# ruizhecao96/CMGAN

Measured on AMD Instinct MI355X. Metric: enhanced audio frames/sec (16 kHz, 2 s clips, batch 32 per GPU), higher is better.
Workload: dtype f32 storage/accumulate; products as 3 x f16 split MFMA (fp32-class accuracy); 1 GPU; configs[1]: batch=32 x 2 s synthetic 16 kHz noisy clips per GPU, n_fft=400 hop=100, TSCNet(64,201) random-init, full pipeline wav->wav; mfma_mode=f16x3, launch=hipGraph replay, batch_per_gpu=32, global_batch=32, frames_per_clip=321, parallelism=dp1

## Files before the change

cmgan_amd/csrc/api.hip:

```cpp
#include <math.h>
#include <stdarg.h>
#include <stdio.h>
#include <string.h>

#include <algorithm>
#include <map>
#include <string>
#include <vector>

#include "api_internal.h"
#include "weights.h"

extern "C" void cmgan_default_config(cmgan_config* c) {
    if (!c) return;
    c->n_fft = 400; c->hop = 100; c->num_features = 201; c->num_channel = 64; c->num_tscb = 4;
    c->heads = 4; c->dim_head = 16; c->conv_kernel = 31; c->max_pos_emb = 512;
    c->mfma_mode = CMGAN_MFMA_F16X3;
    c->single_mask = 0;
}

extern "C" int cmgan_abi_version(void) { return CMGAN_ABI_VERSION; }

extern "C" const char* cmgan_last_error(const cmgan_handle* h) {
    return h ? h->err.c_str() : g_create_error.c_str();
// ... 494 lines not shown
    w.qkv_w = W(h, WID(g, CF_QKV_W), ok);   w.qkv_b = W(h, WID(g, CF_QKV_B), ok);
    w.wo = W(h, WID(g, CF_WO), ok);         w.bo = W(h, WID(g, CF_BO), ok);
    w.rel = W(h, WID(g, CF_REL), ok);
    w.pw1_w = W(h, WID(g, CF_PW1_W), ok);   w.pw1_b = W(h, WID(g, CF_PW1_B), ok);
    w.dw_w = W(h, WID(g, CF_DW_W), ok);     w.dw_b = W(h, WID(g, CF_DW_B), ok);
    w.pw2_w = W(h, WID(g, CF_PW2_W), ok);   w.pw2_b = W(h, WID(g, CF_PW2_B), ok);
    w.ff2_w1 = W(h, WID(g, CF_FF2_W1), ok); w.ff2_b1 = W(h, WID(g, CF_FF2_B1), ok);
    w.ff2_w2 = W(h, WID(g, CF_FF2_W2), ok); w.ff2_b2 = W(h, WID(g, CF_FF2_B2), ok);
    w.post_gb = W(h, WID(g, CF_POST_GB), ok);
    w.max_pos = h->cfg.max_pos_emb;
    return ok;
}

#ifndef CX_IMG
#define CX_IMG 1
#endif
#ifndef CX_NIMG
#define CX_NIMG 1
#endif
struct WsPlan {
    size_t total = 0;
    size_t e[5];
    size_t img[3];
    size_t xa, xb, q, k, v, o, u, w;
    size_t dm, dc;
    size_t partials;
    size_t ns;
    size_t mstat;
    size_t scale;
    size_t spec;
    size_t est;
    size_t frames;
};

static size_t take(size_t& cur, size_t n) {
    const size_t o = cur;
    cur += (n + 63) & ~(size_t)63;
    return o;
}

static WsPlan plan_ws(const cmgan_config& c, int B, int T) {
    WsPlan p;
    const size_t F = c.num_features, F2 = (F + 1) / 2, W2 = 2 * F2;
    const size_t P = (size_t)T * F, P2 = (size_t)T * F2, M = (size_t)B * P2;
    size_t cur = 0;
    p.e[0] = take(cur, (size_t)B * T * std::max(F, W2) * 64);
    for (int i = 1; i < 5; ++i) p.e[i] = take(cur, (size_t)B * P * 64);
    for (int i = 0; i < 3; ++i)
        p.img[i] = (CX_IMG && c.mfma_mode != CMGAN_MFMA_F32 && i < CX_NIMG) ? take(cur, (size_t)B * P * 64) : 0;
    p.xa = take(cur, M * 64);
    p.xb = take(cur, M * 64);
    const size_t qf = std::max(conf_qkv_floats((int)(B * F2), T), conf_qkv_floats(B * T, (int)F2));
    p.q = take(cur, qf); p.k = take(cur, qf); p.v = take(cur, qf); p.o = take(cur, qf);
    p.u = take(cur, M * 128);
    p.w = take(cur, M * 128);
    p.dm = take(cur, (size_t)B * T * W2 * 4 + 64);
    p.dc = take(cur, (size_t)B * T * W2 * 4 + 64);
    const size_t nt = std::max({(size_t)conv3_ntiles(T, (int)F), (size_t)conv_in_ntiles((int)P),
                                (size_t)conv3x_ntiles(T, (int)F, 64), (size_t)conv3x_ntiles(T, (int)F, 128)});
    p.partials = take(cur, (size_t)B * nt * 128 * 2);
    p.ns = take(cur, (size_t)16 * 2 * B * 64);
    p.mstat = take(cur, (size_t)B * 2);
    p.scale = take(cur, (size_t)B);
    p.spec = take(cur, (size_t)B * 2 * P);
    p.est = take(cur, (size_t)B * 2 * P);
    p.frames = take(cur, (size_t)B * T * c.n_fft);
    p.total = cur;
    return p;
}

extern "C" size_t cmgan_workspace_bytes(const cmgan_handle* h, int B, int T) {
    if (!h || B <= 0 || T <= 0) return 0;
    return plan_ws(h->cfg, B, T).total * sizeof(float);
}

extern "C" int cmgan_num_frames(const cmgan_handle* h, int L) { return h ? L / h->cfg.hop + 1 : 0; }

static int check_wave_len(cmgan_handle* h, int L, bool whole_hops) {
// ... 24 lines not shown
    if (!h) return CMGAN_E_BADARG;
    if (!re || !im || !wav_out || B <= 0 || T < 2) return fail(h, CMGAN_E_BADARG, "cmgan_uncompress_istft: bad argument");
    const WsPlan p = plan_ws(h->cfg, B, T);
    if (int rc = check_ws(h, ws, ws_bytes, p.total * sizeof(float))) return rc;
    launch_uncompress_istft(begin(h, stream), h->st, re, im, scale, B, T, (float*)ws + p.frames, wav_out);
    return check_launch(h, "uncompress_istft");
}

extern "C" int cmgan_power_compress(cmgan_handle* h, const float* x, int B, int F, int T, float* y, void* stream) {
    if (!h) return CMGAN_E_BADARG;
    if (!x || !y || B <= 0 || F <= 0 || T <= 0) return fail(h, CMGAN_E_BADARG, "cmgan_power_compress: bad argument");
    launch_power_compress(begin(h, stream), x, B, F, T, y);
    return check_launch(h, "power_compress");
}

extern "C" int cmgan_power_uncompress(cmgan_handle* h, const float* re, const float* im, int B, int F, int T,
                                      float* y, void* stream) {
    if (!h) return CMGAN_E_BADARG;
    if (!re || !im || !y || B <= 0 || F <= 0 || T <= 0) return fail(h, CMGAN_E_BADARG, "cmgan_power_uncompress: bad argument");
    launch_power_uncompress(begin(h, stream), re, im, B, F, T, y);
    return check_launch(h, "power_uncompress");
}

struct ConfPlan { size_t total, xa, xb, q, k, v, o, u, w; };
static ConfPlan plan_conf(int N, int L) {
    ConfPlan p;
    size_t cur = 0;
    const size_t M = (size_t)N * L, qf = conf_qkv_floats(N, L);
    p.xa = take(cur, M * 64); p.xb = take(cur, M * 64);
    p.q = take(cur, qf); p.k = take(cur, qf); p.v = take(cur, qf); p.o = take(cur, qf);
    p.u = take(cur, M * 128); p.w = take(cur, M * 128);
    p.total = cur;
    return p;
}

extern "C" size_t cmgan_conformer_workspace_bytes(const cmgan_handle* h, int N, int L) {
    if (!h || N <= 0 || L <= 0) return 0;
    return plan_conf(N, L).total * sizeof(float);
}

static int conformer_forward_impl(cmgan_handle* h, int index, const float* x, int N, int L, const unsigned char* mask,
                                  float* y, float* taps, void* ws, size_t ws_bytes, void* stream);

static bool conformer_mix(cmgan_handle* h, LaunchCtx ctx, const ConfWeights& w, const ConfWeightsX3& w16, const ConfBuffers& b,
                          const TokMap& seq, long M, float* taps, bool outer_residual, const unsigned char* mask) {
    const int sm = h->cfg.single_mask;
    if (sm == 0) return conformer_forward_x3(ctx, w, w16, b, seq, M, taps, outer_residual, mask);
    if (sm == CMGAN_MIX_ALL || (sm | CMGAN_MIX_CONV) == CMGAN_MIX_ALL)
        return conformer_forward_x1(ctx, w, w16, b, seq, M, taps, outer_residual, mask);
    if (!conformer_x3_addressable(seq)) return false;
    const ConfStageTbl &t3 = conf_stages_x3(), &t1 = conf_stages_x1();
    auto pick = [&](int bit) -> const ConfStageTbl& { return (sm & bit) ? t1 : t3; };
    return conformer_forward_tbl(ctx, pick(CMGAN_MIX_FF1), pick(CMGAN_MIX_QKV), pick(CMGAN_MIX_ATTN), pick(CMGAN_MIX_PW1),
                                 pick(CMGAN_MIX_DWPW2), pick(CMGAN_MIX_FF2), w, w16, b, seq, M, taps, outer_residual, mask);
// ... 5 lines not shown
}

extern "C" int cmgan_conformer_forward_masked(cmgan_handle* h, int index, const float* x, int N, int L,
                                              const unsigned char* mask, float* y, float* taps, void* ws,
                                              size_t ws_bytes, void* stream) {
    if (h && !mask) return fail(h, CMGAN_E_BADARG, "cmgan_conformer_forward_masked: mask is null");
    return conformer_forward_impl(h, index, x, N, L, mask, y, taps, ws, ws_bytes, stream);
}

static int conformer_forward_impl(cmgan_handle* h, int index, const float* x, int N, int L, const unsigned char* mask,
                                  float* y, float* taps, void* ws, size_t ws_bytes, void* stream) {
    if (!h) return CMGAN_E_BADARG;
    if (!x || !y || N <= 0 || L <= 0 || index < 0 || index >= 8) return fail(h, CMGAN_E_BADARG, "cmgan_conformer_forward: bad argument");
    if ((long)N * L >= (1l << 31)) return fail(h, CMGAN_E_BADARG, "cmgan_conformer_forward: N x L too large");
    const TokMap seq = make_seq_map(N, L, 1, L, 0, 1);
    if (h->cfg.mfma_mode != CMGAN_MFMA_F32 && !conformer_x3_addressable(seq))
        return fail(h, CMGAN_E_BADARG, "cmgan_conformer_forward: N x L too large for the split-f16 kernels "
                                       "(L < 2^23, N * ceil(L / 32) < 2^31)");
    const ConfPlan p = plan_conf(N, L);
    if (int rc = check_ws(h, ws, ws_bytes, p.total * sizeof(float))) return rc;
    ConfWeights w;
    if (!conf_weights(h, index, w)) return CMGAN_E_WEIGHTS;
    float* f = (float*)ws;
    ConfBuffers b{f + p.xa, f + p.xb, f + p.q, f + p.k, f + p.v, f + p.o, f + p.u, f + p.w};
    hipStream_t s = (hipStream_t)stream;
    const size_t M = (size_t)N * L;
    HIPCHK(h, hipMemcpyAsync(b.xa, x, M * 64 * sizeof(float), hipMemcpyDeviceToDevice, s));
    if (h->cfg.mfma_mode != CMGAN_MFMA_F32) {
        ConfWeightsX3 w16;
        if (!conf_weights_x3(h, index, w16)) return CMGAN_E_WEIGHTS;
        if (!conformer_mix(h, begin(h, stream), w, w16, b, seq, (long)M, taps, false, mask))
            return fail(h, CMGAN_E_BADARG, "cmgan_conformer_forward: N x L too large for the split-f16 kernels");
    } else {
        conformer_forward(begin(h, stream), w, b, seq, (long)M, taps, false, mask);
    }
    HIPCHK(h, hipMemcpyAsync(y, b.xa, M * 64 * sizeof(float), hipMemcpyDeviceToDevice, s));
    return check_launch(h, "conformer_forward");
}

struct DenseW { const float *w[4], *bias[4], *gb[4], *prelu[4]; const _Float16* w16[4]; };
static bool dense_weights(cmgan_handle* h, int grp, DenseW& d) {
    bool ok = true;
    for (int i = 0; i < 4; ++i) {
        d.w[i] = W(h, WID(grp, DB_W(i)), ok); d.bias[i] = W(h, WID(grp, DB_BIAS(i)), ok);
        d.gb[i] = W(h, WID(grp, DB_GB(i)), ok); d.prelu[i] = W(h, WID(grp, DB_PRELU(i)), ok);
        d.w16[i] = W16(h, WID(grp, DB_W(i)), ok);
    }
// ... 137 lines not shown
    {
        float* slots[4] = {f + p.e[1], f + p.e[2], f + p.e[3], f + p.e[4]};
        float* sc[4] = {nsc(1), nsc(2), nsc(3), nsc(4)};
        float* sh[4] = {nsh(1), nsh(2), nsh(3), nsh(4)};
        float* imgs[3] = {f + p.img[0], f + p.img[1], f + p.img[2]};
        run_dense_block(ctx, x3, dbe, f + p.e[0], nsc(0), nsh(0), c1pr, slots, partials, sc, sh, B, T, F, x3 ? imgs : nullptr, conv3x, frozen,
                        run, 1);
    }
    {
        ConvArgs a{};
        a.in[0] = f + p.e[4]; a.nscale[0] = nsc(4); a.nshift[0] = nsh(4); a.nalpha[0] = dbe.prelu[3];
        a.nslots = 1; a.w = c2w; a.bias = c2b; a.out = f + p.xb; a.partials = partials;
        a.T = T; a.F = F; a.dil = 1; a.mode = 1; a.ntiles = x3 ? conv3x_ntiles(T, F, 64) : conv3_ntiles(T, F);
        if (x3) conv3x(ctx, a, c2w16, B, 1, 64);
        else launch_conv3(ctx, a, B, 1, 64);
        finalize(5, a.ntiles, 64, 0, (double)P2, c2gb, f + p.xb, F2);
        launch_in_apply(ctx, f + p.xb, nsc(5), nsh(5), c2pr, f + p.xa, B, P2);
    }
    if (taps && taps->encoder_dev) launch_cl_to_nchw(ctx, f + p.xa, taps->encoder_dev, B, P2);
    }
    const size_t x_bytes = (size_t)M * 64 * sizeof(float);
    if (opt.x_io && !ph_enc) HIPCHK(h, hipMemcpyAsync(f + p.xa, opt.x_io, x_bytes, hipMemcpyDeviceToDevice, hs));

    ConfBuffers cb{f + p.xa, f + p.xb, f + p.q, f + p.k, f + p.v, f + p.o, f + p.u, f + p.w};
    const TokMap tmap = make_seq_map(B * F2, T, F2, (long)T * F2, 1, F2);
    const TokMap fmap = make_seq_map(B * T, F2, 1, F2, 0, 1);
    for (int k = 0; ph_tscb && k < h->cfg.num_tscb; ++k) {
        if (x3) {
            if (!conformer_x(ctx, cw[2 * k], cw16[2 * k], cb, tmap, M, nullptr, true, nullptr) ||
                !conformer_x(ctx, cw[2 * k + 1], cw16[2 * k + 1], cb, fmap, M, nullptr, true, nullptr))
                return fail(h, CMGAN_E_BADARG, "tscnet_forward: B x T x F too large for the split-f16 conformer kernels "
                                               "(conformer_x3_addressable, conformer_x3.hip)");
        } else {
            conformer_forward(ctx, cw[2 * k], cb, tmap, M, nullptr, true);
            conformer_forward(ctx, cw[2 * k + 1], cb, fmap, M, nullptr, true);
        }
        if (taps && taps->tscb_dev[k]) launch_cl_to_nchw(ctx, f + p.xa, taps->tscb_dev[k], B, P2);
    }

    if (opt.x_io && !ph_dec) HIPCHK(h, hipMemcpyAsync(opt.x_io, f + p.xa, x_bytes, hipMemcpyDeviceToDevice, hs));
    const size_t enc_floats = (size_t)6 * 2 * B * 64;
    if (!ph_dec) {
        if (opt.stats_out && ph_enc)
            HIPCHK(h, hipMemcpyAsync(opt.stats_out, f + p.ns, enc_floats * sizeof(float), hipMemcpyDeviceToDevice, hs));
        return check_launch(h, "tscnet_forward");
    }

// ... 303 lines not shown
```

cmgan_amd/csrc/attn32_x3.hip:

```cpp
#if defined(X3_SINGLE) && defined(A32_STAMP)
#undef A32_STAMP
#endif
#include "kernels.h"
#include <string.h>
#include <stdlib.h>

namespace X3_NS {

typedef float f32x16 __attribute__((ext_vector_type(16)));

__device__ __forceinline__ f32x16 mfma3216(f16x8 a, f16x8 b, f32x16 c) {
    return __builtin_amdgcn_mfma_f32_32x32x16_f16(a, b, c, 0, 0, 0);
}
__device__ __forceinline__ f32x16 mfma3216l(f16x8 a, f16x8 b, f32x16 c) {
    return X3_TERMS == 3 ? __builtin_amdgcn_mfma_f32_32x32x16_f16(a, b, c, 0, 0, 0) : c;
}
__device__ __forceinline__ f32x16 zero16() {
    f32x16 z;
#pragma unroll
    for (int i = 0; i < 16; ++i) z[i] = 0.f;
    return z;
}
#ifdef A32_STAMP
#define A32_SLOTS 2048
// ... 32 lines not shown
    const float a = xchg32(v, b);
    return a + b;
}

#ifndef XCD_ORDER
#define XCD_ORDER 1
#endif
#define XNTB 2
#define XWAVES 8

__device__ __forceinline__ void ln_split32(const f32x4 (&x)[4], f16x8 (&bh)[2], f16x8 (&bl)[2]) {
    float mean, rstd;
    ln_stats(x, mean, rstd);
    f32x4 xh[4];
#pragma unroll
    for (int kb = 0; kb < 4; ++kb) xh[kb] = (x[kb] - splat4(mean)) * splat4(rstd);
    split8(xh[0], xh[1], bh[0], bl[0]);
    split8(xh[2], xh[3], bh[1], bl[1]);
}

__global__ __launch_bounds__(512) void qkv32_x3_kernel(const float* __restrict__ x, TokMap m, int Lt,
                                                       const _Float16* __restrict__ wi, const float* __restrict__ b,
                                                       _Float16* __restrict__ qimg, _Float16* __restrict__ kimg,
                                                       _Float16* __restrict__ vimg, int ntiles) {
    __shared__ __attribute__((aligned(16))) _Float16 wlds[24576];
    __shared__ float scratch[XWAVES * 32 * 17];
    __shared__ __attribute__((aligned(16))) float bias_l[192];
    stage_lds16<3072, 512>(wi, wlds);
    for (int i = threadIdx.x; i < 192; i += blockDim.x) bias_l[i] = b[i];
    __syncthreads();
    const int lane = threadIdx.x & 63, c = lane & 15, g = lane >> 4, wv = threadIdx.x >> 6;
    const int row32 = lane & 31, hh = lane >> 5;
    float* T = scratch + wv * (32 * 17);

#pragma unroll 1
    for (int tile = blockIdx.x * XWAVES + wv; tile < ntiles; tile += gridDim.x * XWAVES) {
        const int n = tile / Lt, it = tile - n * Lt;
        f16x8 xbh[XNTB][2], xbl[XNTB][2];
#pragma unroll
        for (int tb = 0; tb < XNTB; ++tb) {
            int l = it * 32 + tb * 16 + c;
            if (l >= m.L) l = m.L - 1;
            const long row = (long)(n / m.inner) * m.outer + (long)(n % m.inner) * m.istride + (long)l * m.lstride;
            f32x4 xr[4];
#pragma unroll
            for (int kb = 0; kb < 4; ++kb) xr[kb] = ldg4(x + row * 64 + 16 * kb + 4 * g);
            ln_split32(xr, xbh[tb], xbl[tb]);
        }
#pragma unroll 2
        for (int ob = 0; ob < 12; ++ob) {
            const f32x4 bias = *reinterpret_cast<const f32x4*>(&bias_l[16 * ob + 4 * g]);
            f32x4 acc[XNTB];
#pragma unroll
            for (int tb = 0; tb < XNTB; ++tb) acc[tb] = bias;
            lin_acc_x3<2, XNTB>(wlds + ob * 2048 + lane * 8, xbh, xbl, acc);
            const int which = ob >> 2, h = ob & 3;
            const long nh = (long)n * 4 + h;
            if (which < 2) {
                _Float16* img = (which == 0 ? qimg : kimg) + (nh * Lt + it) * 1024;
#pragma unroll
                for (int tb = 0; tb < XNTB; ++tb) {
                    f16x4 hi, lo;
                    split4(acc[tb], hi, lo);
                    _Float16* p = img + ((g >> 1) * 32 + 16 * tb + c) * 8 + 4 * (g & 1);
                    *reinterpret_cast<f16x4*>(p) = hi;
                    *reinterpret_cast<f16x4*>(p + 512) = lo;
                }
            } else {
                wave_lds_fence();
#pragma unroll
                for (int tb = 0; tb < XNTB; ++tb)
#pragma unroll
                    for (int r = 0; r < 4; ++r) T[(16 * tb + c) * 17 + 4 * g + r] = acc[tb][r];
                wave_lds_fence();
#pragma unroll
                for (int grp = 0; grp < 2; ++grp) {
                    f32x4 va, vb;
#pragma unroll
                    for (int r = 0; r < 4; ++r) {
                        va[r] = T[(16 * grp + 4 * hh + r) * 17 + (row32 & 15)];
// ... 645 lines not shown
    ASP_SB();
#pragma unroll
    for (int jt = 0; jt < NF; ++jt)
        if (ASP_ABL != 5 && ASP_ABL != 10) sn[jt] = asp_eq(kh[jt], kl[jt], qh, ql, sn[jt]);
    if (LASTQ) asp_load_q(c, tn.so, tn.it, qh, ql);
    if (ASP_ABL != 1 && ASP_ABL != 7 && ASP_ABL != 10) {
#pragma unroll
        for (int jt = 0; jt < 2; ++jt) asp_load_k(c, tn.so, nn, jt, kh[jt], kl[jt]);
    }
    ASP_FMARK(5);
    ASP_SB();
    if (LG > 3) asp_pv(o, va[3], ph[1], pl[1]);
    if (ASP_ABL != 1 && ASP_ABL != 7 && ASP_ABL != 10) va[3] = asp_load_v(c, tv.so, vn, 3);
    st.l += psum;
    float mx = 0.f;
    if (HOTMX && ASP_ABL != 9) mx = asp_max<2, true>(c, sn, 0);
    ASP_FMARK(6);
#ifdef A32_STAMP
    ++sp.chunks;
#endif
    return mx;
}

template <bool CLAMP, int NKTL, bool FULLL, int TAILK = 0>
__global__ __launch_bounds__(256, ASP_OCC) void attn_sp_out_x3_kernel(const _Float16* __restrict__ qimg,
                                                                const _Float16* __restrict__ kimg,
                                                                const _Float16* __restrict__ vimg,
                                                                const _Float16* __restrict__ eimg, int max_pos,
                                                                float* __restrict__ x, TokMap m,
                                                                const _Float16* __restrict__ woi,
                                                                const float* __restrict__ bo, int Lt, int tpb, int nseq,
                                                                int group, unsigned lt_magic) {
    __shared__ __attribute__((aligned(16))) float rbuf[4][ASP_RFL];
    __shared__ __attribute__((aligned(16))) f32x4 stash[2][4][2][64];
#ifdef A32_STAMP
    A32Stamp sp;
    sp.t = __builtin_readcyclecounter();
    sp.chunks = 0;
#pragma unroll
    for (int i = 0; i < 16; ++i) sp.acc[i] = 0;
#endif
    const int lane = threadIdx.x & 63, wv = __builtin_amdgcn_readfirstlane(threadIdx.x >> 6);
    const int xcd = XCD_ORDER ? (int)(blockIdx.x & 7) : 0, li = XCD_ORDER ? (int)(blockIdx.x >> 3) : (int)blockIdx.x;
    const int nbx = XCD_ORDER ? (int)(gridDim.x >> 3) : (int)gridDim.x;
    const int grp = li / group, gleft = nbx - grp * group;
    const int gs = gleft < group ? gleft : group;
    const int GN = nseq * Lt;
    const int G0 = (xcd * nbx + grp * group) * tpb + (li - grp * group);
    if (G0 >= GN) return;
    const int nleft = (GN - 1 - G0) / gs + 1;
    const int ntl = nleft < tpb ? nleft : tpb;
    auto div_lt = [&](int G) -> int {
        if (__builtin_expect(lt_magic == 0u, 0)) {
            asm volatile("; division path");
            return __builtin_amdgcn_readfirstlane((int)((unsigned)G / (unsigned)Lt));
        }
        return (int)__umulhi((unsigned)__builtin_amdgcn_readfirstlane(G), lt_magic);
// ... 20 lines not shown
    const unsigned seq_bytes = (unsigned)Lt * 8192u;
    const unsigned xstride = (unsigned)m.lstride * 256u, xlane = (unsigned)g16 * 16u;
    const _Float16* wp = woi + wv * 2048 + lane * 8;
    auto tile_of = [&](int G) -> AspTile {
        G = G < GN ? G : GN - 1;
        const int n = div_lt(G);
        AspTile t;
        t.it = G - n * Lt;
        t.so = (unsigned)(n - n0) * seq_bytes;
        return t;
    };

    f16x8 qh, ql, eh[3], el[3], kh[2], kl[2], va[4];
    {
        const AspTile t0 = tile_of(G0);
        asp_load_q(c, t0.so, t0.it, qh, ql);
#pragma unroll
        for (int t = 0; t < 3; ++t) asp_load_e<CLAMP>(c, 32 * t0.it, 0, t, eh[t], el[t]);
#pragma unroll
        for (int jt = 0; jt < 2; ++jt) asp_load_k(c, t0.so, 0, jt, kh[jt], kl[jt]);
#pragma unroll
        for (int g4 = 0; g4 < 4; ++g4) va[g4] = asp_load_v(c, t0.so, 0, g4);
    }
    const int nfull = L >> 6, tail = L & 63;
    const int nch = nfull + (tail ? 1 : 0);

    A32State st;
    st.m = 0.f; st.run = -INFINITY; st.l = 0.f;
    f32x16 o = zero16(), negm = zero16();
    f32x16 s[2];
    if (nch == 1) asp_front<NKTL, CLAMP, true>(c, tile_of(G0 + gs), 0, qh, ql, eh, el, kh, kl, negm, s);
    else asp_front<2, CLAMP, false>(c, tile_of(G0), 1, qh, ql, eh, el, kh, kl, negm, s);

    ASP_CMARK(0);
#pragma unroll 1
    for (int tl = 0; tl < ntl; ++tl) {
        const int G = G0 + tl * gs;
        const AspTile tc = tile_of(G), t1 = tile_of(G + gs);
        const int i0 = 32 * tc.it;
        const int n = n0 + (int)(tc.so / seq_bytes);
        const int nq = __builtin_amdgcn_readfirstlane(n / m.inner);
        char* xbase = reinterpret_cast<char*>(x + ((long)nq * m.outer + (long)(n - nq * m.inner) * m.istride) * 64 + 16 * wv);
        if (nch > 1) asp_reference<2, true>(c, s, 0, st, o, negm);
        else asp_reference<NKTL, FULLL, TAILK>(c, s, 0, st, o, negm);
        int ch = 0;
        while (ch < nch - 2) {
            bool drifted, odd = false;
// ... 3 lines not shown
                float mx = asp_fused<2, 2, true, CLAMP, false, true>(c, tc, ch + 2, tc, ch + 1, qh, ql, eh, el, kh, kl, va, negm, s, sn,
                                                               st, o A32_STAMP_PASS);
                st.run = fmaxf(st.run, mx);
                drifted = __any(st.run > A32_HI || st.run < A32_LO);
                ++ch;
                if (!(ch < nch - 2) || drifted) { odd = true; break; }
                ASP_FMARK(0);
                mx = asp_fused<2, 2, true, CLAMP, false, true>(c, tc, ch + 2, tc, ch + 1, qh, ql, eh, el, kh, kl, va, negm, sn, s, st,
                                                         o A32_STAMP_PASS);
                st.run = fmaxf(st.run, mx);
                drifted = __any(st.run > A32_HI || st.run < A32_LO);
                ++ch;
            } while (ch < nch - 2 && !drifted);
            if (odd) { s[0] = sn[0]; s[1] = sn[1]; }
            if (drifted) asp_reference<2, true>(c, s, 0, st, o, negm);
        }
        if (ch < nch - 1) {
            f32x16 sn[2];
            asp_fused<NKTL, 2, false, CLAMP, true>(c, t1, 0, tc, nch - 1, qh, ql, eh, el, kh, kl, va, negm, s, sn,
                                                   st, o A32_STAMP_PASS);
            asp_reference<NKTL, FULLL, TAILK>(c, sn, 64 * nfull, st, o, negm);
            s[0] = sn[0]; s[1] = sn[1];
        }
        unsigned xo[2];
        f32x4 xold[2], bias;
#pragma unroll
        for (int i = 0; i < 2; ++i) {
            const int l = i0 + 16 * i + c16;
            xo[i] = (unsigned)(l < L ? l : L - 1) * xstride + xlane;
            if (!CLAMP) xold[i] = *reinterpret_cast<const f32x4*>(xbase + xo[i]);
        }
        if (!CLAMP) bias = ldg4(bo + 16 * wv + 4 * g16);
        f32x16 sn[2];
        if (tl + 1 < ntl) {
            const f32x16 zero = zero16();
            if (nch == 1) asp_fused<NKTL, NKTL, false, CLAMP, true, false, TAILK>(c, tile_of(G + 2 * gs), 0, t1, 0, qh, ql, eh, el, kh, kl, va, zero, s, sn, st, o A32_STAMP_PASS);
            else asp_fused<2, NKTL, false, CLAMP, false, true, TAILK>(c, t1, 1, t1, 0, qh, ql, eh, el, kh, kl, va, zero, s, sn, st, o A32_STAMP_PASS);
        } else {
            asp_back<NKTL, TAILK>(s, st, o, va);
        }
        ASP_CMARK(1);
        if (CLAMP) {
#pragma unroll
            for (int i = 0; i < 2; ++i) xold[i] = *reinterpret_cast<const f32x4*>(xbase + xo[i]);
            bias = ldg4(bo + 16 * wv + 4 * g16);
        }
        const f16x8 ah0 = *reinterpret_cast<const f16x8*>(wp), al0 = *reinterpret_cast<const f16x8*>(wp + 512);
        const f16x8 ah1 = *reinterpret_cast<const f16x8*>(wp + 1024), al1 = *reinterpret_cast<const f16x8*>(wp + 1536);
        const float inv = __builtin_amdgcn_rcpf(red_h_sum(st.l));
        f32x4 oa, ob;
#pragma unroll
        for (int r = 0; r < 4; ++r) {
            oa[r] = (o[r] + o[8 + r]) * inv;
            ob[r] = (o[4 + r] + o[12 + r]) * inv;
        }
        const int par = tl & 1;
        stash[par][wv][c.a >> 4][c.hh * 16 + (c.a & 15)] = oa;
        stash[par][wv][c.a >> 4][(2 + c.hh) * 16 + (c.a & 15)] = ob;
        st.m = 0.f; st.run = -INFINITY; st.l = 0.f;
        o = zero16(); negm = zero16();
        s[0] = sn[0]; s[1] = sn[1];
        if (ASP_ABL == 11) {
            if (i0 + c16 < L) asm volatile("global_store_dwordx4 %0, %1, %2\n\ts_nop 1" ::"v"(xo[0]), "v"(oa + ob + xold[0] + bias), "s"(xbase) : "memory");
            continue;
        }
        ASP_CMARK(2);
        __syncthreads();
        ASP_CMARK(3);
#pragma unroll
        for (int i = 0; i < 2; ++i) {
            f16x8 bh0, bl0, bh1, bl1;
// ... 8 lines not shown
            acc = mfma32l(al1, bh1, acc);
            const f32x4 xnew = xold[i] + acc;
            if (i0 + 16 * i + c16 < L)
                asm volatile("global_store_dwordx4 %0, %1, %2\n\ts_nop 1" ::"v"(xo[i]), "v"(xnew), "s"(xbase) : "memory");
        }
        ASP_CMARK(4);
    }
#ifdef A32_STAMP
    ASP_FMARK(0);
    if (lane == 0) {
        const int b = L < 200 ? 32 : 0;
        unsigned long long* slot = g_a32_stamp[(blockIdx.x * 4 + (threadIdx.x >> 6)) & (A32_SLOTS - 1)];
#pragma unroll
        for (int i = 0; i < 16; ++i) atomicAdd(&slot[b + i], sp.acc[i]);
        atomicAdd(&slot[b + 16], 1ull);
        atomicAdd(&slot[b + 17], (unsigned long long)sp.chunks);
    }
#endif
}

}
using namespace X3_NS;

void launch_qkv32_x3(LaunchCtx ctx, const float* x, const TokMap& seq, const _Float16* wi, const float* b,
                     _Float16* qimg, _Float16* kimg, _Float16* vimg) {
    const int N = seq.nblocks / seq.Lb, Lt = (seq.L + 31) / 32;
    const int ntiles = N * Lt;
    const int want = (ntiles + XWAVES - 1) / XWAVES;
    const int grid = want < 512 ? (want > 0 ? want : 1) : 512;
    LAUNCH(ctx, "qkv", (qkv32_x3_kernel<<<grid, 512, 0, ctx.stream>>>(x, seq, Lt, wi, b, qimg, kimg, vimg, ntiles)));
}

void launch_attn32_out_x3(LaunchCtx ctx, const _Float16* qimg, const _Float16* kimg, const _Float16* vimg,
                          const _Float16* rel_img, int max_pos, float* x, const TokMap& seq, const _Float16* woi,
                          const float* bo, const unsigned char* mask) {
    const int N = seq.nblocks / seq.Lb, Lt = (seq.L + 31) / 32;
    const int bps = (Lt + A32_TPB - 1) / A32_TPB;
    const int tpb = (Lt + bps - 1) / bps;
    const long nb = (long)N * bps;
    const unsigned grid = XCD_ORDER ? (unsigned)(((nb + 7) / 8) * 8) : (unsigned)nb;
    LAUNCH(ctx, "attn_out", (attn32_out_x3_kernel<true><<<grid, 256, 0, ctx.stream>>>(
                                qimg, kimg, vimg, rel_img, max_pos, x, seq, woi, bo, Lt, tpb, bps, nb, mask)));
}

#ifndef A32_GROUP_SHORT
#define A32_GROUP_SHORT A32_GROUP
#endif
#ifndef A32_ALIGN_SHORT
#define A32_ALIGN_SHORT 0
#endif
void launch_attn_sp_out_x3(LaunchCtx ctx, const _Float16* qimg, const _Float16* kimg, const _Float16* vimg,
                           const _Float16* rel_img, int max_pos, float* x, const TokMap& seq, const _Float16* woi,
                           const float* bo) {
    const int N = seq.nblocks / seq.Lb, Lt = (seq.L + 31) / 32;
    static const int k_tpb_long = env_knob("CMGAN_ASP_TPB_LONG", A32_TPB, 1, 64), k_group_long = env_knob("CMGAN_ASP_GROUP_LONG", A32_GROUP, 1, 4096);
    static const int k_group_short = env_knob("CMGAN_ASP_GROUP_SHORT", A32_GROUP_SHORT, 1, 4096);
    static const int k_align_short = env_knob("CMGAN_ASP_ALIGN_SHORT", A32_ALIGN_SHORT, 0, 1);
    static const int k_slots = env_knob("CMGAN_ASP_SLOTS", A32_SLOTS_PER_GPU, 8, 65536);
    int tpb = Lt <= 4 ? A32_TPB_SHORT : k_tpb_long;
    if (Lt <= 4 || A32_PERSIST_LONG) {
        const long share = ((long)N * Lt + k_slots - 1) / k_slots;
        if (share > tpb) tpb = (int)share;
        if (Lt <= 4 && k_align_short) tpb = (tpb + Lt - 1) / Lt * Lt;
    }
    const int group = Lt <= 4 ? k_group_short : k_group_long;
    const unsigned lt_magic = Lt > 1 && (long)N * Lt * Lt < (1l << 32) ? (unsigned)((1ul << 32) / (unsigned long)Lt) + 1u : 0u;
    const long nb = ((long)N * Lt + tpb - 1) / tpb;
    const unsigned grid = XCD_ORDER ? (unsigned)(((nb + 7) / 8) * 8) : (unsigned)nb;
    const int tail = seq.L & 63;
    const bool clamp = seq.L + 96 > max_pos;
#define ASP_LAUNCH(CL, NK, FU, ...)                                                                               \
    LAUNCH(ctx, "attn_out", (attn_sp_out_x3_kernel<CL, NK, FU, ##__VA_ARGS__><<<grid, 256, 0, ctx.stream>>>(      \
                                qimg, kimg, vimg, rel_img, max_pos, x, seq, woi, bo, Lt, tpb, N, group, lt_magic)))
    if (!clamp) {
        static const int k_tailk = env_knob("CMGAN_ASP_TAILK", 1, 0, 1);
        if (tail == 0) ASP_LAUNCH(false, 2, true);
        else if (k_tailk && tail == 1) ASP_LAUNCH(false, 1, false, 1);
        else if (k_tailk && tail == 37) ASP_LAUNCH(false, 2, false, 37);
        else if (k_tailk && tail == 45) ASP_LAUNCH(false, 2, false, 45);
        else if (tail > 32) ASP_LAUNCH(false, 2, false);
        else ASP_LAUNCH(false, 1, false);
    } else {
        if (tail == 0) ASP_LAUNCH(true, 2, true);
        else if (tail > 32) ASP_LAUNCH(true, 2, false);
        else ASP_LAUNCH(true, 1, false);
    }
#undef ASP_LAUNCH
}
```

cmgan_amd/csrc/conformer.hip:

```cpp
#include "kernels.h"

#define NTB 2

template <bool FINAL>
__global__ __launch_bounds__(256) void ffn_kernel(const float* xin, float* xout,
                                                  const float* x0,
                                                  const float* __restrict__ post_gb,
                                                  const float* __restrict__ w1, const float* __restrict__ b1,
                                                  const float* __restrict__ w2, const float* __restrict__ b2,
                                                  long M, int nblocks) {
    const int lane = threadIdx.x & 63, c = lane & 15, g = lane >> 4;
    const int wave = blockIdx.x * 4 + (threadIdx.x >> 6);
    const int blk0 = wave * NTB;
    if (blk0 >= nblocks) return;

    long row[NTB];
    bool ok[NTB];
    f32x4 x[NTB][4], xh[NTB][4];
#pragma unroll
    for (int tb = 0; tb < NTB; ++tb) {
        const long t = (long)(blk0 + tb) * 16 + c;
        ok[tb] = t < M;
        row[tb] = ok[tb] ? t : M - 1;
#pragma unroll
// ... 474 lines not shown
    }
}

TokMap make_flat_map(long M) {
    TokMap m{};
    m.seq = 0;
    m.M = M;
    m.nblocks = (int)((M + 15) / 16);
    m.L = 0; m.Lb = 1; m.inner = 1; m.outer = 0; m.istride = 0; m.lstride = 0;
    return m;
}

TokMap make_seq_map(int N, int L, int inner, long outer, long istride, long lstride) {
    TokMap m{};
    m.seq = 1;
    m.L = L;
    m.Lb = (L + 15) / 16;
    m.nblocks = N * m.Lb;
    m.M = 0;
    m.inner = inner; m.outer = outer; m.istride = istride; m.lstride = lstride;
    return m;
}

size_t conf_qkv_floats(int N, int L) { return (size_t)N * 4 * (2 * ((L + 31) / 32)) * 256; }

static inline int grid_for_blocks(int nblocks) {
    const int waves = (nblocks + NTB - 1) / NTB;
    return (waves + 3) / 4;
}

void launch_dwconv(LaunchCtx ctx, const float* u, float* out, const float* dw_w, const float* dw_b, const TokMap& seq) {
    const int N = seq.nblocks / seq.Lb;
    dim3 dwgrid(N, (seq.L + DW_TL - 1) / DW_TL);
    LAUNCH(ctx, "dwconv", (dwconv_kernel<<<dwgrid, 256, 0, ctx.stream>>>(u, out, dw_w, dw_b, seq)));
}

void conformer_forward(LaunchCtx ctx, const ConfWeights& w, const ConfBuffers& b, const TokMap& seq, long M,
                       float* taps, bool outer_residual, const unsigned char* mask) {
    const TokMap flat = make_flat_map(M);
    const int N = seq.nblocks / seq.Lb;
    hipStream_t s = ctx.stream;
    const size_t tap_bytes = (size_t)M * 64 * sizeof(float);

    LAUNCH(ctx, "ffn", (ffn_kernel<false><<<grid_for_blocks(flat.nblocks), 256, 0, s>>>(
                           b.xa, b.xb, nullptr, nullptr, w.ff1_w1, w.ff1_b1, w.ff1_w2, w.ff1_b2, M,
                           flat.nblocks)));
// ... 72 lines not shown
```

cmgan_amd/csrc/conformer_x3.hip:

```cpp
#include "kernels.h"
#include <stdlib.h>
#ifndef FFN32_DEFAULT
#define FFN32_DEFAULT 1
#endif

namespace X3_NS {

#define XNTB 2
#define XWAVES 8
#ifndef FFN_WAVES
#define FFN_WAVES 12
#endif
#ifdef X3_SINGLE
#define FFN_POST_WAVES 8
#else
#define FFN_POST_WAVES FFN_WAVES
#endif

__device__ __forceinline__ float swish_x(float hp) { return swish_scaled(hp); }

__device__ __forceinline__ void ln_split(const f32x4 (&x)[4], f16x8 (&bh)[2], f16x8 (&bl)[2]) {
    float mean, rstd;
    ln_stats(x, mean, rstd);
    f32x4 xh[4];
// ... 670 lines not shown
}

static void stage_ffn(LaunchCtx ctx, int ff, bool plain, const float* xin, float* xout, const float* x0, const ConfWeights& w,
                      const ConfWeightsX3& w16, long M) {
    static const bool k_ffn32 = env_knob("CMGAN_FFN32", FFN32_DEFAULT, 0, 1) != 0;
    const int flat_tiles = (int)(((M + 15) / 16 + XNTB - 1) / XNTB);
    hipStream_t s = ctx.stream;
    const bool final_ = ff == 2 && !plain;
    const _Float16 *w1 = ff == 1 ? w16.ff1_w1 : w16.ff2_w1, *w2 = ff == 1 ? w16.ff1_w2 : w16.ff2_w2;
    const _Float16 *w1_32 = ff == 1 ? w16.ff1_w1_32 : w16.ff2_w1_32, *w2_32 = ff == 1 ? w16.ff1_w2_32 : w16.ff2_w2_32;
    const float *b1 = ff == 1 ? w.ff1_b1 : w.ff2_b1, *b2 = ff == 1 ? w.ff1_b2 : w.ff2_b2;
    if (k_ffn32) { launch_ffn32_x3(ctx, final_, xin, xout, final_ ? x0 : nullptr, final_ ? w.post_gb : nullptr, w1_32, b1, w2_32, b2, M); return; }
    if (final_)
        LAUNCH(ctx, "ffn_post", (ffn_x3_kernel<true, 2, FFN_POST_WAVES><<<ffn_grid(flat_tiles, FFN_POST_WAVES), 64 * FFN_POST_WAVES, 0, s>>>(
                                    xin, xout, x0, w.post_gb, w1, b1, w2, b2, M, flat_tiles)));
    else
        LAUNCH(ctx, "ffn", (ffn_x3_kernel<false, 2, FFN_WAVES><<<ffn_grid(flat_tiles), 64 * FFN_WAVES, 0, s>>>(
                               xin, xout, nullptr, nullptr, w1, b1, w2, b2, M, flat_tiles)));
}

static void stage_qkv(LaunchCtx ctx, const float* x, const TokMap& seq, const ConfWeights& w, const ConfWeightsX3& w16,
                      const ConfBuffers& b) {
    launch_qkv32_x3(ctx, x, seq, w16.qkv_w, w.qkv_b, reinterpret_cast<_Float16*>(b.q), reinterpret_cast<_Float16*>(b.k),
                    reinterpret_cast<_Float16*>(b.v));
}

static void stage_attn(LaunchCtx ctx, float* x, const TokMap& seq, const ConfWeights& w, const ConfWeightsX3& w16,
                       const ConfBuffers& b, const unsigned char* mask) {
    const _Float16 *qimg = reinterpret_cast<const _Float16*>(b.q), *kimg = reinterpret_cast<const _Float16*>(b.k),
                   *vimg = reinterpret_cast<const _Float16*>(b.v);
    if (!mask) launch_attn_sp_out_x3(ctx, qimg, kimg, vimg, w16.rel_planes, w.max_pos, x, seq, w16.wo, w.bo);
    else launch_attn32_out_x3(ctx, qimg, kimg, vimg, w16.rel_planes, w.max_pos, x, seq, w16.wo, w.bo, mask);
}

static void stage_pw1glu(LaunchCtx ctx, const float* x, const ConfWeights& w, const ConfWeightsX3& w16, const ConfBuffers& b,
                         long M) {
    const int flat_tiles = (int)(((M + 15) / 16 + XNTB - 1) / XNTB);
    LAUNCH(ctx, "pw1glu", (pw1glu_x3_kernel<<<persistent_grid(flat_tiles, 2), 512, 0, ctx.stream>>>(
                              x, b.u, w16.pw1_w, w.pw1_b, M, flat_tiles)));
}

static void stage_dwpw2(LaunchCtx ctx, float* x, const TokMap& seq, const ConfWeights& w, const ConfWeightsX3& w16,
                        const ConfBuffers& b) {
    const int N = seq.nblocks / seq.Lb;
    const int ntl = (seq.L + DP_TL - 1) / DP_TL;
    const int nsegs = (ntl + DS_SEG - 1) / DS_SEG;
    const long items = (long)N * nsegs;
#if DS_TOEPLITZ
    const unsigned pgrid = items < 512 ? (unsigned)(((items + 7) / 8) * 8) : 512u;
    LAUNCH(ctx, "dwpw2", (dwpw2t_x3_kernel<<<pgrid, 512, 0, ctx.stream>>>(x, b.u, w16.dw_img, w.dw_b, w16.pw2_w, w.pw2_b, seq, N,
                                                                         nsegs)));
#else
    const unsigned grid = XCD_ORDER ? (unsigned)(((items + 7) / 8) * 8) : (unsigned)items;
    LAUNCH(ctx, "dwpw2", (dwpw2s_x3_kernel<<<grid, 256, 0, ctx.stream>>>(x, b.u, w.dw_w, w.dw_b, w16.pw2_w, w.pw2_b, seq, N,
// ... 40 lines not shown
```

cmgan_amd/csrc/kernels.h:

```cpp
#pragma once
#include <hip/hip_runtime.h>
#include <vector>
#include "common.hip.h"

struct Profiler {
    bool enabled = false;
    struct Rec { const char* name; hipEvent_t a, b; };
    std::vector<Rec> recs;
    std::vector<hipEvent_t> pool;
    size_t used = 0;
    hipEvent_t get() {
        if (used == pool.size()) { hipEvent_t e; hipEventCreate(&e); pool.push_back(e); }
        return pool[used++];
    }
    void reset() { recs.clear(); used = 0; }
};

struct Fork {
    int count = 0, at = 0;
    bool fired = false;
    hipEvent_t ev = nullptr;
    void tick(hipStream_t s) {
        if (!fired && ++count >= at) { hipEventRecord(ev, s); fired = true; }
    }
// ... 82 lines not shown
                      const float* gw, float* dm, int B, int T, int Fe);
void launch_mask_stats(LaunchCtx, const float* dm, const float* scalars, int B, int T, int F, float* mstat);
void launch_final_combine(LaunchCtx, const float* spec, const float* dm, const float* dc, const float* mstat,
                          const float* mk_scalars, const float* prelu_out, const float* cx_bias,
                          int B, int T, int F, float* out_re, float* out_im, float* tap_mask, float* tap_cplx);
void launch_cl_to_nchw(LaunchCtx, const float* in, float* out, int B, long P);

void launch_in_running(LaunchCtx, const float* x, int B, int T, int PF, int hist, double* part, size_t part_doubles,
                       double* sums, const float* gb, float* nscale, float* nshift);
void launch_mask_running(LaunchCtx, const float* dm, const float* scalars, int B, int T, int F, int hist,
                         double* part, size_t part_doubles, double* sums, float* mstat);

struct ConfWeights {
    const float *ff1_w1, *ff1_b1, *ff1_w2, *ff1_b2;
    const float *qkv_w, *qkv_b, *wo, *bo, *rel;
    const float *pw1_w, *pw1_b, *dw_w, *dw_b, *pw2_w, *pw2_b;
    const float *ff2_w1, *ff2_b1, *ff2_w2, *ff2_b2, *post_gb;
    int max_pos;
};
struct ConfBuffers {
    float *xa, *xb;
    float *q, *k, *v, *o;
    float *u, *w;
};
TokMap make_flat_map(long M);
TokMap make_seq_map(int N, int L, int inner, long outer, long istride, long lstride);
size_t conf_qkv_floats(int N, int L);
void conformer_forward(LaunchCtx, const ConfWeights&, const ConfBuffers&, const TokMap& seq, long M, float* taps,
                       bool outer_residual, const unsigned char* mask = nullptr);

struct ConfWeightsX3 {
    const _Float16 *ff1_w1, *ff1_w2, *qkv_w, *wo, *pw1_w, *pw2_w, *ff2_w1, *ff2_w2;
    const _Float16* rel_img;
    const _Float16* dw_img;
    const _Float16* rel_planes;
    const _Float16 *ff1_w1_32, *ff1_w2_32, *ff2_w1_32, *ff2_w2_32;
};
void launch_ffn32_x3(LaunchCtx, bool final_, const float* xin, float* xout, const float* x0, const float* post_gb,
                     const _Float16* w1i, const float* b1, const _Float16* w2i, const float* b2, long M);
struct ConfStageTbl {
    void (*ffn)(LaunchCtx, int ff, bool plain, const float* xin, float* xout, const float* x0, const ConfWeights&,
                const ConfWeightsX3&, long M);
    void (*qkv)(LaunchCtx, const float* x, const TokMap& seq, const ConfWeights&, const ConfWeightsX3&, const ConfBuffers&);
    void (*attn)(LaunchCtx, float* x, const TokMap& seq, const ConfWeights&, const ConfWeightsX3&, const ConfBuffers&,
                 const unsigned char* mask);
    void (*pw1glu)(LaunchCtx, const float* x, const ConfWeights&, const ConfWeightsX3&, const ConfBuffers&, long M);
    void (*dwpw2)(LaunchCtx, float* x, const TokMap& seq, const ConfWeights&, const ConfWeightsX3&, const ConfBuffers&);
};
const ConfStageTbl& conf_stages_x3();
const ConfStageTbl& conf_stages_x1();
bool conformer_forward_tbl(LaunchCtx, const ConfStageTbl& ff1, const ConfStageTbl& qkv, const ConfStageTbl& attn,
                           const ConfStageTbl& pw1, const ConfStageTbl& dwpw2, const ConfStageTbl& ff2,
                           const ConfWeights&, const ConfWeightsX3&, const ConfBuffers&, const TokMap& seq, long M,
                           float* taps, bool outer_residual, const unsigned char* mask);
bool conformer_x3_addressable(const TokMap& seq);
bool conformer_forward_x3(LaunchCtx, const ConfWeights&, const ConfWeightsX3&, const ConfBuffers&, const TokMap& seq,
                          long M, float* taps, bool outer_residual, const unsigned char* mask = nullptr);
void launch_dwconv(LaunchCtx, const float* u, float* out, const float* dw_w, const float* dw_b, const TokMap& seq);
void launch_qkv32_x3(LaunchCtx, const float* x, const TokMap& seq, const _Float16* wi, const float* b,
                     _Float16* qimg, _Float16* kimg, _Float16* vimg);
void launch_attn32_out_x3(LaunchCtx, const _Float16* qimg, const _Float16* kimg, const _Float16* vimg,
                          const _Float16* rel_img, int max_pos, float* x, const TokMap& seq, const _Float16* woi,
                          const float* bo, const unsigned char* mask);
void launch_attn_sp_out_x3(LaunchCtx, const _Float16* qimg, const _Float16* kimg, const _Float16* vimg,
                           const _Float16* rel_img, int max_pos, float* x, const TokMap& seq, const _Float16* woi,
                           const float* bo);
int  conv3x_ntiles(int T, int F, int cout);
void launch_conv3_x3(LaunchCtx, const ConvArgs&, const void* w16, int B, int time_taps, int cout);
void launch_conv3_x3_dgrad(LaunchCtx, const ConvArgs&, const void* w16, int B);
void launch_selftest_x3(hipStream_t, const void* a_img, const float* b_fm, float* d, int M32);

void launch_selftest_mfma(hipStream_t, const float* a_fm, const float* b_fm, float* d, int KB);

bool conformer_forward_x1(LaunchCtx, const ConfWeights&, const ConfWeightsX3&, const ConfBuffers&, const TokMap& seq,
                          long M, float* taps, bool outer_residual, const unsigned char* mask = nullptr);
void launch_qkv32_x1(LaunchCtx, const float* x, const TokMap& seq, const _Float16* wi, const float* b,
                     _Float16* qimg, _Float16* kimg, _Float16* vimg);
void launch_attn32_out_x1(LaunchCtx, const _Float16* qimg, const _Float16* kimg, const _Float16* vimg,
                          const _Float16* rel_img, int max_pos, float* x, const TokMap& seq, const _Float16* woi,
                          const float* bo, const unsigned char* mask);
void launch_attn_sp_out_x1(LaunchCtx, const _Float16* qimg, const _Float16* kimg, const _Float16* vimg,
                           const _Float16* rel_img, int max_pos, float* x, const TokMap& seq, const _Float16* woi,
                           const float* bo);
void launch_conv3_x1(LaunchCtx, const ConvArgs&, const void* w16, int B, int time_taps, int cout);
void launch_ffn32_x1(LaunchCtx, bool final_, const float* xin, float* xout, const float* x0, const float* post_gb,
                     const _Float16* w1i, const float* b1, const _Float16* w2i, const float* b2, long M);
#ifdef X3_SINGLE
#define X3_NS x1k
#define conformer_forward_x3 conformer_forward_x1
#define conformer_x3_addressable conformer_x1_addressable
#define conf_stages_x3 conf_stages_x1
#define launch_qkv32_x3 launch_qkv32_x1
#define launch_attn32_out_x3 launch_attn32_out_x1
#define launch_attn_sp_out_x3 launch_attn_sp_out_x1
#define launch_conv3_x3 launch_conv3_x1
#define launch_ffn32_x3 launch_ffn32_x1
#else
#define X3_NS x3k
#endif
```

Before: 488,500 frames/s.

## Handle the lone trailing key of L%64==1 attention in the epilogue

Result: no change. 490,500 frames/s, median of 6 (+0.4%).

```diff
diff --git a/cmgan_amd/csrc/api.hip b/cmgan_amd/csrc/api.hip
--- a/cmgan_amd/csrc/api.hip
+++ b/cmgan_amd/csrc/api.hip
@@ -540,7 +540,7 @@
     size_t total = 0;
     size_t e[5];
     size_t img[3];
-    size_t xa, xb, q, k, v, o, u, w;
+    size_t xa, xb, q, k, v, o, u, w, lone;
     size_t dm, dc;
     size_t partials;
     size_t ns;
@@ -572,6 +572,7 @@
     p.q = take(cur, qf); p.k = take(cur, qf); p.v = take(cur, qf); p.o = take(cur, qf);
     p.u = take(cur, M * 128);
     p.w = take(cur, M * 128);
+    p.lone = take(cur, conf_lone_floats((int)std::max(B * F2, (size_t)B * T)));
     p.dm = take(cur, (size_t)B * T * W2 * 4 + 64);
     p.dc = take(cur, (size_t)B * T * W2 * 4 + 64);
     const size_t nt = std::max({(size_t)conv3_ntiles(T, (int)F), (size_t)conv_in_ntiles((int)P),
@@ -642,7 +643,7 @@
     return check_launch(h, "power_uncompress");
 }
 
-struct ConfPlan { size_t total, xa, xb, q, k, v, o, u, w; };
+struct ConfPlan { size_t total, xa, xb, q, k, v, o, u, w, lone; };
 static ConfPlan plan_conf(int N, int L) {
     ConfPlan p;
     size_t cur = 0;
@@ -650,6 +651,7 @@
     p.xa = take(cur, M * 64); p.xb = take(cur, M * 64);
     p.q = take(cur, qf); p.k = take(cur, qf); p.v = take(cur, qf); p.o = take(cur, qf);
     p.u = take(cur, M * 128); p.w = take(cur, M * 128);
+    p.lone = take(cur, conf_lone_floats(N));
     p.total = cur;
     return p;
 }
@@ -701,7 +703,7 @@
     ConfWeights w;
     if (!conf_weights(h, index, w)) return CMGAN_E_WEIGHTS;
     float* f = (float*)ws;
-    ConfBuffers b{f + p.xa, f + p.xb, f + p.q, f + p.k, f + p.v, f + p.o, f + p.u, f + p.w};
+    ConfBuffers b{f + p.xa, f + p.xb, f + p.q, f + p.k, f + p.v, f + p.o, f + p.u, f + p.w, f + p.lone};
     hipStream_t s = (hipStream_t)stream;
     const size_t M = (size_t)N * L;
     HIPCHK(h, hipMemcpyAsync(b.xa, x, M * 64 * sizeof(float), hipMemcpyDeviceToDevice, s));
@@ -885,7 +887,7 @@
     const size_t x_bytes = (size_t)M * 64 * sizeof(float);
     if (opt.x_io && !ph_enc) HIPCHK(h, hipMemcpyAsync(f + p.xa, opt.x_io, x_bytes, hipMemcpyDeviceToDevice, hs));
 
-    ConfBuffers cb{f + p.xa, f + p.xb, f + p.q, f + p.k, f + p.v, f + p.o, f + p.u, f + p.w};
+    ConfBuffers cb{f + p.xa, f + p.xb, f + p.q, f + p.k, f + p.v, f + p.o, f + p.u, f + p.w, f + p.lone};
     const TokMap tmap = make_seq_map(B * F2, T, F2, (long)T * F2, 1, F2);
     const TokMap fmap = make_seq_map(B * T, F2, 1, F2, 0, 1);
     for (int k = 0; ph_tscb && k < h->cfg.num_tscb; ++k) {
diff --git a/cmgan_amd/csrc/attn32_x3.hip b/cmgan_amd/csrc/attn32_x3.hip
--- a/cmgan_amd/csrc/attn32_x3.hip
+++ b/cmgan_amd/csrc/attn32_x3.hip
@@ -78,7 +78,7 @@
 __global__ __launch_bounds__(512) void qkv32_x3_kernel(const float* __restrict__ x, TokMap m, int Lt,
                                                        const _Float16* __restrict__ wi, const float* __restrict__ b,
                                                        _Float16* __restrict__ qimg, _Float16* __restrict__ kimg,
-                                                       _Float16* __restrict__ vimg, int ntiles) {
+                                                       _Float16* __restrict__ vimg, float* __restrict__ lone, int ntiles) {
     __shared__ __attribute__((aligned(16))) _Float16 wlds[24576];
     __shared__ float scratch[XWAVES * 32 * 17];
     __shared__ __attribute__((aligned(16))) float bias_l[192];
@@ -112,6 +112,7 @@
             lin_acc_x3<2, XNTB>(wlds + ob * 2048 + lane * 8, xbh, xbl, acc);
             const int which = ob >> 2, h = ob & 3;
             const long nh = (long)n * 4 + h;
+            if (lone && which >= 1 && it == Lt - 1 && c == 0) stg4(lone + nh * 32 + 16 * (which - 1) + 4 * g, acc[0]);
             if (which < 2) {
                 _Float16* img = (which == 0 ? qimg : kimg) + (nh * Lt + it) * 1024;
 #pragma unroll
@@ -803,7 +804,7 @@
     return mx;
 }
 
-template <bool CLAMP, int NKTL, bool FULLL, int TAILK = 0>
+template <bool CLAMP, int NKTL, bool FULLL, int TAILK = 0, bool LONE = false>
 __global__ __launch_bounds__(256, ASP_OCC) void attn_sp_out_x3_kernel(const _Float16* __restrict__ qimg,
                                                                 const _Float16* __restrict__ kimg,
                                                                 const _Float16* __restrict__ vimg,
@@ -811,9 +812,12 @@
                                                                 float* __restrict__ x, TokMap m,
                                                                 const _Float16* __restrict__ woi,
                                                                 const float* __restrict__ bo, int Lt, int tpb, int nseq,
-                                                                int group, unsigned lt_magic) {
+                                                                int group, unsigned lt_magic, int Lk,
+                                                                const float* __restrict__ lone) {
+    static_assert(!LONE || (FULLL && NKTL == 2 && TAILK == 0 && !CLAMP), "LONE rides on the L % 64 == 0 instantiation");
     __shared__ __attribute__((aligned(16))) float rbuf[4][ASP_RFL];
     __shared__ __attribute__((aligned(16))) f32x4 stash[2][4][2][64];
+    __shared__ __attribute__((aligned(16))) float lone_l[LONE ? 4 : 1][32];
 #ifdef A32_STAMP
     A32Stamp sp;
     sp.t = __builtin_readcyclecounter();
@@ -880,7 +884,7 @@
 #pragma unroll
         for (int g4 = 0; g4 < 4; ++g4) va[g4] = asp_load_v(c, t0.so, 0, g4);
     }
-    const int nfull = L >> 6, tail = L & 63;
+    const int nfull = Lk >> 6, tail = Lk & 63;
     const int nch = nfull + (tail ? 1 : 0);
 
     A32State st;
@@ -930,6 +934,7 @@
             asp_reference<NKTL, FULLL, TAILK>(c, sn, 64 * nfull, st, o, negm);
             s[0] = sn[0]; s[1] = sn[1];
         }
+        constexpr bool BLATE = CLAMP || LONE;
         unsigned xo[2];
         f32x4 xold[2], bias;
 #pragma unroll
@@ -938,7 +943,12 @@
             xo[i] = (unsigned)(l < L ? l : L - 1) * xstride + xlane;
             if (!CLAMP) xold[i] = *reinterpret_cast<const f32x4*>(xbase + xo[i]);
         }
-        if (!CLAMP) bias = ldg4(bo + 16 * wv + 4 * g16);
+        if (!BLATE) bias = ldg4(bo + 16 * wv + 4 * g16);
+        float lv = 0.f;
+        if (LONE) {
+            const float* lp = lone + ((long)n * 4 + wv) * 32;
+            lv = lp[(unsigned)c.a];
+        }
         f32x16 sn[2];
         if (tl + 1 < ntl) {
             const f32x16 zero = zero16();
@@ -951,10 +961,40 @@
         if (CLAMP) {
 #pragma unroll
             for (int i = 0; i < 2; ++i) xold[i] = *reinterpret_cast<const f32x4*>(xbase + xo[i]);
-            bias = ldg4(bo + 16 * wv + 4 * g16);
-        }
+        }
+        f16x8 q2h, q2l, e2h, e2l;
+        if (LONE) {
+            asp_load_q(c, tc.so, tc.it, q2h, q2l);
+            const unsigned ev = (unsigned)c.hh * (c.eplane2 >> 1) + (unsigned)(max_pos + L - 1 - i0 - c.a) * 16u;
+            e2h = buf_h8(c.er, ev, 0);
+            e2l = buf_h8(c.er, ev, c.eplane2);
+        }
+        if (BLATE) bias = ldg4(bo + 16 * wv + 4 * g16);
         const f16x8 ah0 = *reinterpret_cast<const f16x8*>(wp), al0 = *reinterpret_cast<const f16x8*>(wp + 512);
         const f16x8 ah1 = *reinterpret_cast<const f16x8*>(wp + 1024), al1 = *reinterpret_cast<const f16x8*>(wp + 1536);
+        if (LONE) {
+            lone_l[wv][c.a] = lv;
+            wave_lds_fence();
+            const f32x4 k0 = *reinterpret_cast<const f32x4*>(&lone_l[wv][8 * c.hh]);
+            const f32x4 k1 = *reinterpret_cast<const f32x4*>(&lone_l[wv][8 * c.hh + 4]);
+            const f32x4 v0 = *reinterpret_cast<const f32x4*>(&lone_l[wv][16 + 4 * c.hh]);
+            const f32x4 v1 = *reinterpret_cast<const f32x4*>(&lone_l[wv][24 + 4 * c.hh]);
+            float sh = 0.f;
+#pragma unroll
+            for (int e = 0; e < 8; ++e)
+                sh += ((float)q2h[e] + (float)q2l[e]) * ((e < 4 ? k0[e] : k1[e - 4]) + ((float)e2h[e] + (float)e2l[e]));
+            const float d = red_h_sum(sh) - st.m;
+            const float ex = __builtin_amdgcn_exp2f(-fabsf(d));
+            const float sc = d > 0.f ? ex : 1.0f, p = d > 0.f ? 1.0f : ex;
+            st.l = st.l * sc + (c.hh ? 0.f : p);
+#pragma unroll
+            for (int v = 0; v < 16; ++v) o[v] *= sc;
+#pragma unroll
+            for (int r = 0; r < 4; ++r) {
+                o[r] += p * v0[r];
+                o[4 + r] += p * v1[r];
+            }
+        }
         const float inv = __builtin_amdgcn_rcpf(red_h_sum(st.l));
         f32x4 oa, ob;
 #pragma unroll
@@ -1009,13 +1049,15 @@
 }
 using namespace X3_NS;
 
+static bool asp_lone_len(int L) { return L % 64 == 1 && L >= 65; }
 void launch_qkv32_x3(LaunchCtx ctx, const float* x, const TokMap& seq, const _Float16* wi, const float* b,
-                     _Float16* qimg, _Float16* kimg, _Float16* vimg) {
+                     _Float16* qimg, _Float16* kimg, _Float16* vimg, float* lone) {
     const int N = seq.nblocks / seq.Lb, Lt = (seq.L + 31) / 32;
     const int ntiles = N * Lt;
     const int want = (ntiles + XWAVES - 1) / XWAVES;
     const int grid = want < 512 ? (want > 0 ? want : 1) : 512;
-    LAUNCH(ctx, "qkv", (qkv32_x3_kernel<<<grid, 512, 0, ctx.stream>>>(x, seq, Lt, wi, b, qimg, kimg, vimg, ntiles)));
+    if (!asp_lone_len(seq.L)) lone = nullptr;
+    LAUNCH(ctx, "qkv", (qkv32_x3_kernel<<<grid, 512, 0, ctx.stream>>>(x, seq, Lt, wi, b, qimg, kimg, vimg, lone, ntiles)));
 }
 
 void launch_attn32_out_x3(LaunchCtx ctx, const _Float16* qimg, const _Float16* kimg, const _Float16* vimg,
@@ -1036,9 +1078,12 @@
 #ifndef A32_ALIGN_SHORT
 #define A32_ALIGN_SHORT 0
 #endif
+#ifndef ASP_LONEKEY_DEFAULT
+#define ASP_LONEKEY_DEFAULT 1
+#endif
 void launch_attn_sp_out_x3(LaunchCtx ctx, const _Float16* qimg, const _Float16* kimg, const _Float16* vimg,
                            const _Float16* rel_img, int max_pos, float* x, const TokMap& seq, const _Float16* woi,
-                           const float* bo) {
+                           const float* bo, const float* lone) {
     const int N = seq.nblocks / seq.Lb, Lt = (seq.L + 31) / 32;
     static const int k_tpb_long = env_knob("CMGAN_ASP_TPB_LONG", A32_TPB, 1, 64), k_group_long = env_knob("CMGAN_ASP_GROUP_LONG", A32_GROUP, 1, 4096);
     static const int k_group_short = env_knob("CMGAN_ASP_GROUP_SHORT", A32_GROUP_SHORT, 1, 4096);
@@ -1056,12 +1101,20 @@
     const unsigned grid = XCD_ORDER ? (unsigned)(((nb + 7) / 8) * 8) : (unsigned)nb;
     const int tail = seq.L & 63;
     const bool clamp = seq.L + 96 > max_pos;
+    int Lk = seq.L;
 #define ASP_LAUNCH(CL, NK, FU, ...)                                                                               \
     LAUNCH(ctx, "attn_out", (attn_sp_out_x3_kernel<CL, NK, FU, ##__VA_ARGS__><<<grid, 256, 0, ctx.stream>>>(      \
-                                qimg, kimg, vimg, rel_img, max_pos, x, seq, woi, bo, Lt, tpb, N, group, lt_magic)))
+                                qimg, kimg, vimg, rel_img, max_pos, x, seq, woi, bo, Lt, tpb, N, group, lt_magic, Lk, lone)))
     if (!clamp) {
         static const int k_tailk = env_knob("CMGAN_ASP_TAILK", 1, 0, 1);
-        if (tail == 0) ASP_LAUNCH(false, 2, true);
+        static const int k_lonekey = env_knob("CMGAN_ASP_LONEKEY", ASP_LONEKEY_DEFAULT, 0, 1);
+        if (ASP_ABL == 12 && asp_lone_len(seq.L)) {
+            Lk = seq.L - 1;
+            ASP_LAUNCH(false, 2, true);
+        } else if (k_lonekey && lone && asp_lone_len(seq.L)) {
+            Lk = seq.L - 1;
+            ASP_LAUNCH(false, 2, true, 0, true);
+        } else if (tail == 0) ASP_LAUNCH(false, 2, true);
         else if (k_tailk && tail == 1) ASP_LAUNCH(false, 1, false, 1);
         else if (k_tailk && tail == 37) ASP_LAUNCH(false, 2, false, 37);
         else if (k_tailk && tail == 45) ASP_LAUNCH(false, 2, false, 45);
diff --git a/cmgan_amd/csrc/conformer.hip b/cmgan_amd/csrc/conformer.hip
--- a/cmgan_amd/csrc/conformer.hip
+++ b/cmgan_amd/csrc/conformer.hip
@@ -520,6 +520,7 @@
     return m;
 }
 
+size_t conf_lone_floats(int N) { return (size_t)N * 4 * 32; }
 size_t conf_qkv_floats(int N, int L) { return (size_t)N * 4 * (2 * ((L + 31) / 32)) * 256; }
 
 static inline int grid_for_blocks(int nblocks) {
diff --git a/cmgan_amd/csrc/conformer_x3.hip b/cmgan_amd/csrc/conformer_x3.hip
--- a/cmgan_amd/csrc/conformer_x3.hip
+++ b/cmgan_amd/csrc/conformer_x3.hip
@@ -716,14 +716,14 @@
 static void stage_qkv(LaunchCtx ctx, const float* x, const TokMap& seq, const ConfWeights& w, const ConfWeightsX3& w16,
                       const ConfBuffers& b) {
     launch_qkv32_x3(ctx, x, seq, w16.qkv_w, w.qkv_b, reinterpret_cast<_Float16*>(b.q), reinterpret_cast<_Float16*>(b.k),
-                    reinterpret_cast<_Float16*>(b.v));
+                    reinterpret_cast<_Float16*>(b.v), b.lone);
 }
 
 static void stage_attn(LaunchCtx ctx, float* x, const TokMap& seq, const ConfWeights& w, const ConfWeightsX3& w16,
                        const ConfBuffers& b, const unsigned char* mask) {
     const _Float16 *qimg = reinterpret_cast<const _Float16*>(b.q), *kimg = reinterpret_cast<const _Float16*>(b.k),
                    *vimg = reinterpret_cast<const _Float16*>(b.v);
-    if (!mask) launch_attn_sp_out_x3(ctx, qimg, kimg, vimg, w16.rel_planes, w.max_pos, x, seq, w16.wo, w.bo);
+    if (!mask) launch_attn_sp_out_x3(ctx, qimg, kimg, vimg, w16.rel_planes, w.max_pos, x, seq, w16.wo, w.bo, b.lone);
     else launch_attn32_out_x3(ctx, qimg, kimg, vimg, w16.rel_planes, w.max_pos, x, seq, w16.wo, w.bo, mask);
 }
 
diff --git a/cmgan_amd/csrc/kernels.h b/cmgan_amd/csrc/kernels.h
--- a/cmgan_amd/csrc/kernels.h
+++ b/cmgan_amd/csrc/kernels.h
@@ -128,9 +128,11 @@
     float *xa, *xb;
     float *q, *k, *v, *o;
     float *u, *w;
+    float *lone;
 };
 TokMap make_flat_map(long M);
 TokMap make_seq_map(int N, int L, int inner, long outer, long istride, long lstride);
+size_t conf_lone_floats(int N);
 size_t conf_qkv_floats(int N, int L);
 void conformer_forward(LaunchCtx, const ConfWeights&, const ConfBuffers&, const TokMap& seq, long M, float* taps,
                        bool outer_residual, const unsigned char* mask = nullptr);
@@ -164,13 +166,13 @@
                           long M, float* taps, bool outer_residual, const unsigned char* mask = nullptr);
 void launch_dwconv(LaunchCtx, const float* u, float* out, const float* dw_w, const float* dw_b, const TokMap& seq);
 void launch_qkv32_x3(LaunchCtx, const float* x, const TokMap& seq, const _Float16* wi, const float* b,
-                     _Float16* qimg, _Float16* kimg, _Float16* vimg);
+                     _Float16* qimg, _Float16* kimg, _Float16* vimg, float* lone);
 void launch_attn32_out_x3(LaunchCtx, const _Float16* qimg, const _Float16* kimg, const _Float16* vimg,
                           const _Float16* rel_img, int max_pos, float* x, const TokMap& seq, const _Float16* woi,
                           const float* bo, const unsigned char* mask);
 void launch_attn_sp_out_x3(LaunchCtx, const _Float16* qimg, const _Float16* kimg, const _Float16* vimg,
                            const _Float16* rel_img, int max_pos, float* x, const TokMap& seq, const _Float16* woi,
-                           const float* bo);
+                           const float* bo, const float* lone);
 int  conv3x_ntiles(int T, int F, int cout);
 void launch_conv3_x3(LaunchCtx, const ConvArgs&, const void* w16, int B, int time_taps, int cout);
 void launch_conv3_x3_dgrad(LaunchCtx, const ConvArgs&, const void* w16, int B);
@@ -181,13 +183,13 @@
 bool conformer_forward_x1(LaunchCtx, const ConfWeights&, const ConfWeightsX3&, const ConfBuffers&, const TokMap& seq,
                           long M, float* taps, bool outer_residual, const unsigned char* mask = nullptr);
 void launch_qkv32_x1(LaunchCtx, const float* x, const TokMap& seq, const _Float16* wi, const float* b,
-                     _Float16* qimg, _Float16* kimg, _Float16* vimg);
+                     _Float16* qimg, _Float16* kimg, _Float16* vimg, float* lone);
 void launch_attn32_out_x1(LaunchCtx, const _Float16* qimg, const _Float16* kimg, const _Float16* vimg,
                           const _Float16* rel_img, int max_pos, float* x, const TokMap& seq, const _Float16* woi,
                           const float* bo, const unsigned char* mask);
 void launch_attn_sp_out_x1(LaunchCtx, const _Float16* qimg, const _Float16* kimg, const _Float16* vimg,
                            const _Float16* rel_img, int max_pos, float* x, const TokMap& seq, const _Float16* woi,
-                           const float* bo);
+                           const float* bo, const float* lone);
 void launch_conv3_x1(LaunchCtx, const ConvArgs&, const void* w16, int B, int time_taps, int cout);
 void launch_ffn32_x1(LaunchCtx, bool final_, const float* xin, float* xout, const float* x0, const float* post_gb,
                      const _Float16* w1i, const float* b1, const _Float16* w2i, const float* b2, long M);
```
